# nsfisis/RayTracingInOneWeekend.zig

Hardware: AMD Instinct MI355X
Metric: Msamples/sec (pixels x spp / s), RTIOW cover scene; trace-kernel roofline (higher is better)
Workload: dtype f64; 1 GPU; BASELINE configs[1]: RTIOW cover scene 1200x675, 500 spp per GPU (500 spp frame), depth 50, rows interleaved over 1 GPU(s); width=1200, height=675, spp_frame=500, max_depth=50, seed=42, precision=f64, parallelism=rows1

## Files before the change

### include/rtw_hip.h

```cpp
#ifndef RTW_HIP_H
#define RTW_HIP_H

#include <stddef.h>
#include <stdint.h>

#ifdef __cplusplus
extern "C" {
#endif

#define RTW_ABI_VERSION 4

typedef enum {
  RTW_OK = 0,
  RTW_EINVAL = -1,
  RTW_UNSUPPORTED = -2,
  RTW_EHIP = -3,
  RTW_ENOMEM = -4,
  RTW_ENODEV = -5
} rtw_status;

typedef enum {
  RTW_LAMBERT_SOLID = 0,
  RTW_LAMBERT_CHECKER = 1,
  RTW_METAL = 2,
// ... 92 lines not shown
const char *rtw_last_error(void);

int rtw_camera_init(rtw_camera *cam, const double look_from[3], const double look_at[3],
                    const double vup[3], double vfov, double aspect_ratio, double aperture,
                    double focus_dist, double time0, double time1);
uint32_t rtw_image_height(uint32_t width, double aspect_ratio);
int rtw_cover_scene(uint64_t seed, rtw_sphere *spheres, uint32_t *n_spheres,
                    rtw_material *mats, uint32_t *n_mats, uint64_t rng_state_out[4]);

int rtw_render(const rtw_camera *cam, const rtw_sphere *spheres, uint32_t n_spheres,
               const rtw_material *mats, uint32_t n_mats, const rtw_params *params,
               uint8_t *rgb_out, float *mean_out);

typedef struct rtw_scene_s *rtw_scene;

int rtw_scene_create(const rtw_sphere *spheres, uint32_t n_spheres, const rtw_material *mats,
                     uint32_t n_mats, rtw_scene *out);
int rtw_scene_destroy(rtw_scene scene);

size_t rtw_workspace_bytes(const rtw_params *params);

typedef struct rtw_timer_s *rtw_timer;
int rtw_timer_create(rtw_timer *out);
int rtw_timer_destroy(rtw_timer t);
int rtw_timer_elapsed_ms(rtw_timer t, float *ms);

typedef struct rtw_sclk_probe_s *rtw_sclk_probe;
int rtw_sclk_probe_begin(void *stream, double wall_ms, rtw_sclk_probe *out);
int rtw_sclk_probe_end(rtw_sclk_probe p, double *mhz);

int rtw_render_device(rtw_scene scene, const rtw_camera *cam, const rtw_params *params,
                      void *workspace, size_t workspace_bytes, uint8_t *d_rgb, float *d_mean,
                      void *stream, rtw_timer timer);

int rtw_render_counts(rtw_scene scene, const rtw_camera *cam, const rtw_params *params,
                      void *workspace, size_t workspace_bytes, uint64_t counts_out[4]);
int rtw_render_counts_ex(rtw_scene scene, const rtw_camera *cam, const rtw_params *params,
                         void *workspace, size_t workspace_bytes, uint64_t counts_out[6]);
#define RTW_STATS_WORDS 16
enum {
  RTW_STAT_SAMPLES = 0, RTW_STAT_SEGMENTS = 1, RTW_STAT_F32_SKIPS = 2,
  RTW_STAT_CAND_WAVE_ITERS = 3, RTW_STAT_CAND_LANES = 4, RTW_STAT_DISC_GE0_LANES = 5,
  RTW_STAT_SPHERE_LOOP_WAVE_ITERS = 6, RTW_STAT_CULL_SURVIVOR_LANES = 7, RTW_STAT_CULL_EXACT_WAVE_ITERS = 8,
  RTW_STAT_DRAIN_SEGMENTS = 9, RTW_STAT_DRAIN_SAMPLES = 10, RTW_STAT_CLUSTER_WAVE_TESTS = 11,
  RTW_STAT_CLUSTER_WAVE_SKIPS = 12, RTW_STAT_DRAIN_WAVE_ITERS = 13,
  RTW_STAT_PRIMARY_ROUNDS = 14, RTW_STAT_PRIMARY_IDLE_LANES = 15
};
int rtw_render_stats(rtw_scene scene, const rtw_camera *cam, const rtw_params *params,
                     void *workspace, size_t workspace_bytes, uint64_t stats_out[RTW_STATS_WORDS]);
#define RTW_STATS_WORDS_EX 24
enum {
  RTW_STAT_PRIMARY_MASK_POPCOUNT = 16,
  RTW_STAT_TAIL_HELPED_SAMPLES = 17, RTW_STAT_TAIL_WAVE_ITERS = 18, RTW_STAT_TAIL_IDLE_LANE_ITERS = 19,
  RTW_STAT_UNTRACED_UNITS = 20, RTW_STAT_UNTRACED_SAMPLES = 21
};
int rtw_render_stats_ex(rtw_scene scene, const rtw_camera *cam, const rtw_params *params,
                        void *workspace, size_t workspace_bytes, uint64_t *stats_out, uint32_t n_words);


typedef enum {
  RTW_PRIM_SPHERE = 0,
  RTW_PRIM_MOVING_SPHERE = 1,
  RTW_PRIM_XY_RECT = 2,
  RTW_PRIM_XZ_RECT = 3,
  RTW_PRIM_YZ_RECT = 4
} rtw_prim_kind;

typedef struct {
  uint32_t kind, mat;
  int32_t xform;
  uint32_t reserved;
  double a[9];
} rtw_prim;

#define RTW_MAX_XFORM_OPS 4
typedef enum {
  RTW_XF_TRANSLATE = 0,
  RTW_XF_ROTATE_Y = 1
} rtw_xform_op;
typedef struct {
  uint32_t n;
  uint32_t op[RTW_MAX_XFORM_OPS];
  double v[RTW_MAX_XFORM_OPS][3];
} rtw_xform;

typedef enum {
  RTW_TEX_SOLID = 0,
  RTW_TEX_CHECKER = 1,
  RTW_TEX_NOISE = 2,
  RTW_TEX_IMAGE = 3
} rtw_texture_kind;
typedef struct {
  uint32_t kind, perlin, image, reserved;
  double color[3], odd[3], even[3];
  double scale;
} rtw_texture;

typedef enum {
  RTW_WMAT_LAMBERT = 0,
  RTW_WMAT_METAL = 1,
  RTW_WMAT_DIELECTRIC = 2,
  RTW_WMAT_LIGHT = 3
} rtw_wmaterial_kind;
typedef struct {
  uint32_t kind, tex;
  double albedo[3];
  double fuzz, ir;
// ... 175 lines not shown
```

### raytracinginoneweekend.zig_amd/csrc/rtw_capi.hip

```cpp
#include <hip/hip_runtime.h>

#include <algorithm>
#include <cstdarg>
#include <cstdio>
#include <cstdlib>
#include <cstring>
#include <map>
#include <mutex>
#include <string>
#include <utility>
#include <vector>

#include "rtw_hip.h"
#include "rtw_capi_shared.hpp"
#include "rtw_internal.hpp"
#include "rtw_math.hpp"
#include "rtw_scene_pack.hpp"

namespace {

thread_local std::string g_err;

}

int rtw_fail(int status, const char* fmt, ...) {
  char buf[512];
  va_list ap;
  va_start(ap, fmt);
  vsnprintf(buf, sizeof(buf), fmt, ap);
  va_end(ap);
  g_err = buf;
  return status;
}

namespace {

const char* dev_knob(const char* name) {
#ifdef RTW_MEASURE
  return getenv(name);
#else
  (void)name;
  return nullptr;
#endif
}

uint64_t splitmix_first(uint64_t seed) {
  uint64_t z = seed + 0x9e3779b97f4a7c15ULL;
  z = (z ^ (z >> 30)) * 0xbf58476d1ce4e5b9ULL;
  z = (z ^ (z >> 27)) * 0x94d049bb133111ebULL;
  return z ^ (z >> 31);
}

constexpr int kBpcTail = 16;
struct DevInfo {
  int cus = 0;
  std::map<std::pair<int, bool>, std::pair<size_t, int>> bpc;
};
std::mutex g_dev_mu;
std::map<int, DevInfo> g_dev;

int device_cus(int dev) {
  std::lock_guard<std::mutex> lk(g_dev_mu);
  auto& d = g_dev[dev];
  if (d.cus == 0) {
    int v = 0;
    if (hipDeviceGetAttribute(&v, hipDeviceAttributeMultiprocessorCount, dev) != hipSuccess || v <= 0) v = 256;
    d.cus = v;
// ... 157 lines not shown
  a.chunk = rtwp::eff_chunk(p);
  a.n_chunks = rtwp::n_chunks(p);
  a.row_begin = p->row_begin;
  a.row_stride = p->row_stride;
  a.row_count = p->row_count;
  a.tiles_x = rtwp::tiles_x(p);
  a.total_units = (uint32_t)rtwp::total_units(p);
  const rtwm::UDivMagic mu = rtwm::udiv_magic((uint32_t)rtwp::tile_units(1, a.n_chunks)), mt = rtwm::udiv_magic(a.tiles_x);
  a.upt_m = mu.m, a.upt_sh = mu.sh, a.tx_m = mt.m, a.tx_sh = mt.sh;
  a.seed_base = splitmix_first(p->seed) + seed_adv;
  a.unit_order = unit_order(0u);
  a.empty_on = 0u;
  a.partial = reinterpret_cast<double*>(ws + L.partial_off);
  a.counter = reinterpret_cast<uint32_t*>(ws + L.counter_off);
  a.stats = reinterpret_cast<unsigned long long*>(ws + L.stats_off);
}

size_t lds_bytes(const rtw_scene_s* sc, int prec, uint32_t n_clusters) {
  const size_t r = prec == 1 ? 4 : 8;
  return rtwk::kCoopLdsBytes + r * (8 * ((size_t)sc->n + 1) + (size_t)sc->n + 8 * (size_t)sc->nm + 4 * (size_t)sc->ng) +
         4 * ((size_t)sc->n + 1 + sc->nm + sc->n + rtwk::kClusterSlots * (size_t)n_clusters) + 16;
}

uint32_t clusters_usable(const rtw_scene_s* sc, const rtw_camera* cam) {
  if (!sc->v64.cluster_on) return 0u;
  for (const auto& g : sc->groups)
    if (!(cam->time0 >= g.first && cam->time1 <= g.second)) return 0u;
  return 1u;
}

template <typename R>
int launch_engine(const rtwk::SceneView<R>& view, const rtw_camera* cam, const rtw_params* p, unsigned char* ws,
                  const WsLayout& L, uint64_t seed_adv, const RtwPassMap& map, uint32_t cl_on, int dev, size_t lds,
                  uint32_t grid_cap, hipStream_t stream, int mode, bool masked, size_t tail_lds) {
  rtwk::TraceArgs<R> a;
  fill_args(a, view, cam, p, ws, L, seed_adv);
  map.apply(a);
  a.sc.cluster_on = cl_on;
  if (!cl_on) a.sc.n_clusters = 0u;
  a.primary_on = (p->engine == RTW_ENGINE_MEGAKERNEL && rtwk::trace_primary_first((int)p->precision, masked) &&
                  cl_on && a.sc.n_clusters * rtwk::kClusterSlots <= 64u)
                     ? 1u
                     : 0u;
  a.tail_on = (a.primary_on && tail_lds) ? 1u : 0u;
  const uint32_t n_wide = a.sc.g_static_wide + (a.sc.g_moving_wide - a.sc.g_static);
  a.empty_on = (a.primary_on && a.max_depth >= 1u && a.sc.n_clusters * rtwk::kClusterSlots + n_wide <= 64u) ? 1u : 0u;
  if (const char* ek = dev_knob("RTW_TRACE_EMPTY"); ek && ek[0] == '0') a.empty_on = 0u;
  if (a.tail_on) lds += tail_lds;
  if (p->engine == RTW_ENGINE_WAVEFRONT) {
    if (mode == 2) return rtw_fail(RTW_UNSUPPORTED, "phase profile runs on the megakernel engine");
    return rtw_run_wavefront<R>(a, p, ws, L, dev, lds, stream, mode == 1);
  }
  const uint32_t grid = std::max(1u, std::min(grid_cap, (a.total_units + 255) / 256));
  hipError_t e;
  if constexpr (sizeof(R) == 8)
    e = rtwk::launch_trace_f64(a, grid, lds, stream, mode, masked);
  else
    e = rtwk::launch_trace_f32(a, grid, lds, stream, mode, masked);
  if (e != hipSuccess) return rtw_fail(RTW_EHIP, "trace kernel launch: %s", hipGetErrorString(e));
  return RTW_OK;
}

int launch_all(rtw_scene sc, const rtw_camera* cam, const rtw_params* p, void* workspace, size_t ws_bytes,
               uint8_t* d_rgb, float* d_mean, hipStream_t stream, rtw_timer timer, int mode,
               uint64_t seed_adv = 0, rtw_accum acc = nullptr) {
  const WsLayout L = rtwp::ws_layout(p);
  int dev = 0;
  RtwPassMap map;
  bool launch = true;
  const int st0 = rtw_launch_begin(L, workspace, ws_bytes, sc->device,
                                   "scene lives on device %d but the current device is %d", acc, timer, stream, &dev,
                                   &map, &launch);
  if (st0 != RTW_OK || !launch) return st0;
  auto* ws = static_cast<unsigned char*>(workspace);
  const bool masked = map.list && p->engine == RTW_ENGINE_MEGAKERNEL;
  const uint32_t cl_on = p->precision == RTW_PRECISION_F64 ? clusters_usable(sc, cam) : 0u;
  size_t lds = lds_bytes(sc, (int)p->precision, cl_on ? sc->v64.n_clusters : 0u);
  if (p->engine == RTW_ENGINE_MEGAKERNEL) lds += rtwk::trace_home_lds_bytes((int)p->precision, masked);
  if (lds > 64 * 1024) return rtw_fail(RTW_UNSUPPORTED, "scene tables need %zu B of LDS", lds);
  const int bpc = blocks_per_cu(dev, (int)p->precision, lds, masked);
  const uint32_t grid_cap = (uint32_t)(device_cus(dev) * bpc);
  size_t tail_lds = p->engine == RTW_ENGINE_MEGAKERNEL ? rtwk::trace_tail_lds_bytes((int)p->precision, masked) : 0;
  if (const char* tk = dev_knob("RTW_TRACE_TAIL"); tk && tk[0] == '0') tail_lds = 0;
  if (tail_lds && (lds + tail_lds > 64 * 1024 || blocks_per_cu(dev, (int)p->precision, lds + tail_lds, masked, true) != bpc))
    tail_lds = 0;
  if (timer) HIP_TRY(hipEventRecord(timer->start, stream));
  const int st = p->precision == RTW_PRECISION_F32
                     ? launch_engine(sc->v32, cam, p, ws, L, seed_adv, map, cl_on, dev, lds, grid_cap, stream, mode,
                                     masked, tail_lds)
                     : launch_engine(sc->v64, cam, p, ws, L, seed_adv, map, cl_on, dev, lds, grid_cap, stream, mode,
                                     masked, tail_lds);
  if (st != RTW_OK) return st;
  if (timer) {
    HIP_TRY(hipEventRecord(timer->stop, stream));
    timer->recorded = true;
  }
  if (acc) return rtw_accum_pass_fold(acc, p, ws, stream);
  if (d_rgb) return rtw_launch_finalize(p, ws, d_rgb, d_mean, stream);
  return RTW_OK;
}
}

extern "C" {

size_t rtw_workspace_bytes(const rtw_params* p) {
  if (rtw_validate_params(p) != RTW_OK) return 0;
// ... 327 lines not shown
```

### raytracinginoneweekend.zig_amd/csrc/rtw_device.hpp

```cpp
#pragma once
#include <hip/hip_runtime.h>

#include "rtw_beam.hpp"
#include "rtw_cull.hpp"
#include "rtw_internal.hpp"
#include "rtw_math.hpp"

namespace rtwk {

template <typename R>
struct V3 {
  R x, y, z;
};
template <typename R>
__device__ __forceinline__ V3<R> mk(R x, R y, R z) {
  return V3<R>{x, y, z};
}
template <typename R>
__device__ __forceinline__ V3<R> add(V3<R> a, V3<R> b) {
  return mk(a.x + b.x, a.y + b.y, a.z + b.z);
}
template <typename R>
__device__ __forceinline__ V3<R> sub(V3<R> a, V3<R> b) {
  return mk(a.x - b.x, a.y - b.y, a.z - b.z);
// ... 550 lines not shown
      root = (-hb + sq) / a;
      if (root < tmin || tmax < root) continue;
    }
    tmax = root;
    hit = (int)k;
  }
  (void)l_rad;
}

template <typename R>
struct LdsTables {
  CoopSlots* slots;
  R* sph;
  R* rad;
  R* mat;
  R* tg;
  uint32_t* meta;
  uint32_t* kind;
  uint32_t* perm;
  uint32_t* cpos;
};
template <typename R>
__device__ __forceinline__ LdsTables<R> stage_tables(const SceneView<R>& S, unsigned char* lds_raw) {
  LdsTables<R> T;
  T.slots = reinterpret_cast<CoopSlots*>(lds_raw) + (threadIdx.x >> 6);
  T.sph = reinterpret_cast<R*>(lds_raw + kCoopBytesPerWave * (kTraceBlock / 64));
  T.rad = T.sph + 8 * (S.n + 1);
  T.mat = T.rad + S.n;
  T.tg = T.mat + 8 * S.nm;
  T.meta = reinterpret_cast<uint32_t*>(T.tg + 4 * S.ng);
  T.kind = T.meta + S.n + 1;
  T.perm = T.kind + S.nm;
  T.cpos = T.perm + S.n;
  for (uint32_t i = threadIdx.x; i < 8 * (S.n + 1); i += blockDim.x) T.sph[i] = S.sph[i];
  for (uint32_t i = threadIdx.x; i < S.n; i += blockDim.x) T.rad[i] = S.rad[i];
  for (uint32_t i = threadIdx.x; i < 8 * S.nm; i += blockDim.x) T.mat[i] = S.mat[i];
  for (uint32_t i = threadIdx.x; i < 4 * S.ng; i += blockDim.x) T.tg[i] = S.tg[i];
  for (uint32_t i = threadIdx.x; i < S.n + 1; i += blockDim.x) T.meta[i] = S.meta[i];
  for (uint32_t i = threadIdx.x; i < S.nm; i += blockDim.x) T.kind[i] = S.kind[i];
  for (uint32_t i = threadIdx.x; i < S.n; i += blockDim.x) T.perm[i] = S.perm[i];
  for (uint32_t i = threadIdx.x; i < kClusterSlots * S.n_clusters; i += blockDim.x) T.cpos[i] = S.cpos[i];
  __syncthreads();
  return T;
}

struct KStats {
  unsigned long long samples = 0, segments = 0, skipped = 0;
  unsigned long long candwave = 0, candlane = 0, disc = 0, wave_iters = 0;
  unsigned long long cull_lanes = 0, cull_iters = 0;
  unsigned long long cl_tests = 0, cl_skips = 0;
  unsigned long long prim_rounds = 0, prim_idle = 0, mask_pop = 0;
  unsigned long long tail_helped = 0, tail_iters = 0, tail_idle = 0;
  unsigned long long empty_units = 0, empty_samples = 0;
  uint64_t ph[10] = {0, 0, 0, 0, 0, 0, 0, 0, 0, 0};
  uint64_t t_last = 0;
};
#define RTW_STAMP(slot)                                                          \
  if constexpr (MODE == 2) {                                                     \
    __builtin_amdgcn_sched_barrier(0);                                           \
    uint64_t t_;                                                                 \
    asm volatile("s_memtime %0\n\ts_waitcnt lgkmcnt(0)" : "=s"(t_)::"memory"); \
    __builtin_amdgcn_sched_barrier(0);                                           \
    st.ph[slot] += t_ - st.t_last;                                               \
    st.t_last = t_;                                                              \
  }

template <typename R, bool F32, int MODE, bool PRIMARY = false, bool FLAT = false, typename SV>
__device__ __forceinline__ void closest_hit(const SV& S, const LdsTables<R>& T, const Lane<R>& L, R tmin,
                                            R pre_k, uint32_t lid, KStats& st, int& hit, R& tmax, uint32_t pm0 = 0u,
                                            uint32_t pm1 = 0u) {
  static_assert(!PRIMARY || !F32, "the primary form is f64 only (clustered tables)");
  constexpr bool STATS = MODE == 1;
  const R a = norm2(L.d);
  const R inv_a = (R)1 / a;
  const R pre_lim = pre_k * a;
  int tg_cur = -1;
  R frac = (R)0;
  const RTW_CONST uint32_t* c_meta = cptr(S.meta);
  const RTW_CONST R* c_sph = cptr(S.sph);
  const RTW_CONST R* c_tg = cptr(S.tg);
  int hit_orig = -1;
  bool nan_seen = false;
  auto accept = [&](R root, int pos, int orig) {
    if (root != root) nan_seen = true;
    if (!(root < tmin) & ((root < tmax) | ((root == tmax) & (orig > hit_orig)))) {
      tmax = root;
      hit = pos;
      hit_orig = orig;
    }
  };
  auto test = [&](uint32_t k, uint32_t meta, R cx, R cy, R cz, R r2) {
    const R ocx = L.o.x - cx, ocy = L.o.y - cy, ocz = L.o.z - cz;
    const R hb = ocx * L.d.x + ocy * L.d.y + ocz * L.d.z;
    const R cc = (ocx * ocx + ocy * ocy + ocz * ocz) - r2;
    const R disc = hb * hb - a * cc;
    if (!(disc < (R)0)) {
      const bool pre = (hb > (R)0) & (cc > (R)0) & (hb < pre_lim);
      bool cand = !pre;
      if (F32) cand = cand & ((int)k != L.skip);
      if constexpr (STATS) {
        const uint64_t cm = __ballot(cand);
        if (cm && lid == (uint32_t)__builtin_ctzll(__ballot(true))) st.candwave++;
        st.candlane += cand ? 1 : 0;
        st.disc += 1;
      }
      if (cand) {
// ... 323 lines not shown
```

### raytracinginoneweekend.zig_amd/csrc/rtw_internal.hpp

```cpp
#pragma once
#include <hip/hip_runtime.h>
#include <stdint.h>

#include "rtw_layout.hpp"

namespace rtwk {

constexpr uint32_t kBatch = 64;

template <typename R>
struct SceneView {
  const R* sph;
  const R* rad;
  const uint32_t* meta;
  const R* mat;
  const uint32_t* kind;
  const R* tg;
  const double* wide_d;
  const double* tg_d;
  const uint32_t* perm;
  const float* cull;
  const uint32_t* cull_tg;
  const float* tg_f;
  uint32_t n, nm, ng;
  uint32_t g_static_wide, g_static, g_moving_wide;
  uint32_t nn, nn_pad, n_sn;
  uint32_t cull_on;
  float cull_cmax;
  float cull_rho;
  const float* ccull;
  const uint32_t* ccull_tg;
  const float* cclus;
  const uint32_t* cpos;
  const uint32_t* cvalid;
  uint32_t n_clusters;
  uint32_t cluster_on;
  float cull_rho_cl;
};

template <typename R>
struct TraceArgs {
  SceneView<R> sc;
  R origin[3], horizontal[3], vertical[3], llc[3], cu[3], cv[3];
  R lens_radius, time0, time1;
  R bg[3];
  R tmin;
  R inv_w1, inv_h1;
  R pre_k;
  uint32_t W, H, spp, max_depth, chunk, n_chunks;
  uint32_t row_begin, row_stride, row_count, tiles_x;
  uint32_t total_units;
  uint32_t upt_m, upt_sh, tx_m, tx_sh;
  uint32_t unit_order;
  uint32_t primary_on;
  uint32_t tail_on;
  uint32_t empty_on;
  uint64_t seed_base;
  double* partial;
  uint32_t* counter;
  unsigned long long* stats;
  const uint32_t* tile_list;
  const uint64_t* tile_mask;
};

struct FinalizeArgs {
  const double* partial;
  uint8_t* rgb;
  float* mean;
  uint32_t npix, n_chunks;
  double scale;
};

hipError_t launch_trace_f64(const TraceArgs<double>& a, uint32_t grid, size_t lds, hipStream_t s, int mode,
                            bool masked);
hipError_t launch_trace_f32(const TraceArgs<float>& a, uint32_t grid, size_t lds, hipStream_t s, int mode,
                            bool masked);
hipError_t launch_finalize(const FinalizeArgs& a, hipStream_t s);
int trace_blocks_per_cu(int precision, size_t lds, bool masked);
bool trace_primary_first(int precision, bool masked);
constexpr size_t kHomeLdsBytesPerWave = 2560;
constexpr size_t kPrimaryLdsBytesPerWave = 4 * 64 * 4;
size_t trace_home_lds_bytes(int precision, bool masked);
constexpr int kTraceBlock = 256;
constexpr uint32_t kTailWindow = 4;
constexpr size_t kTailLdsBytesPerWave = (3 + kTailWindow) * 64 * 4;
size_t trace_tail_lds_bytes(int precision, bool masked);

struct FoldArgs {
  const double* partial;
  double* sum;
  double* stat;
  uint32_t npix, n_chunks;
  uint32_t n_full;
};
struct ResolveArgs {
  const double* sum;
  uint8_t* rgb;
  float* mean;
  uint32_t npix;
  double scale;
};
struct NoiseArgs {
  const double* stat;
  double* part;
  uint32_t npix;
  double m;
  double denom;
};
struct MaskedFoldArgs {
  FoldArgs f;
  const uint8_t* act;
  uint32_t* cnt;
  uint32_t pass_spp;
};
struct ActiveArgs {
  uint8_t* act;
  const uint8_t* user;
  const double* stat;
  const uint32_t* cnt;
  uint64_t* tile_mask;
  uint32_t* tile_list;
  uint32_t* n_active;
  uint32_t W, rows, tiles_x, n_tiles;
  uint32_t chunk, min_spp;
  double thr;
  uint32_t done;
  uint32_t from_cnt;
};
struct ResolveCntArgs {
  const double* sum;
  const uint32_t* cnt;
  uint8_t* rgb;
  float* mean;
  uint32_t npix;
// ... 137 lines not shown
```

### raytracinginoneweekend.zig_amd/csrc/rtw_trace.hip

```cpp
#include <hip/hip_runtime.h>

#include <type_traits>

#include "rtw_device.hpp"


namespace rtwk {

template <bool F32, bool MASKED>
struct TraceCfg {
  static constexpr int kWavesPerSimd = (F32 && !MASKED) ? 5 : 4;
  static constexpr bool kLoopArgsFromKernarg = !F32;
  static constexpr bool kPrimaryFirst = !F32 && !MASKED;
  static constexpr size_t kHomeStride = kHomeLdsBytesPerWave + (kPrimaryFirst ? kPrimaryLdsBytesPerWave : 0);
  static constexpr size_t kTailBytes = kPrimaryFirst ? kTailLdsBytesPerWave : 0;
};

template <typename R, bool F32, int MODE, bool MASKED>
__global__ void __launch_bounds__(kTraceBlock, (TraceCfg<F32, MASKED>::kWavesPerSimd)) trace_kernel(TraceArgs<R> A) {
  using Cfg = TraceCfg<F32, MASKED>;
  constexpr bool STATS = MODE == 1;
  extern __shared__ __align__(16) unsigned char lds_raw[];
  const SceneView<R> S = A.sc;
  const LdsTables<R> T = stage_tables<R>(S, lds_raw);
  CoopSlots* slots = T.slots;

  const uint32_t lid = lane_id();
  double* h_sum = nullptr;
  uint32_t* h_u32 = nullptr;
  {
    const size_t off = (size_t)(reinterpret_cast<unsigned char*>(T.cpos + kClusterSlots * S.n_clusters) - lds_raw);
    const size_t stride = Cfg::kHomeStride + (Cfg::kTailBytes != 0 && A.tail_on ? Cfg::kTailBytes : 0);
    unsigned char* hb = lds_raw + ((off + 7) & ~(size_t)7) + (threadIdx.x >> 6) * stride;
    h_sum = reinterpret_cast<double*>(hb);
    h_u32 = reinterpret_cast<uint32_t*>(hb + 3 * 64 * 8);
  }
#define RTW_KA(f) (Cfg::kLoopArgsFromKernarg ? opaque(kargs<R>())->f : A.f)
  const R kInf = (R)__builtin_huge_val();

  Lane<R> L;
  L.px = L.ly = L.s = L.depth = 0;
  L.rs = 0;
  L.skip = -1;
  uint32_t lane_flags = 0u;
  LaneFlag<1u> have_unit{lane_flags};
  LaneFlag<2u> have_ray{lane_flags};
  LaneFlag<4u> done{lane_flags};
  uint32_t qnext = 0, qend = 0;
  KStats st;
  if constexpr (MODE == 2) asm volatile("s_memtime %0\n\ts_waitcnt lgkmcnt(0)" : "=s"(st.t_last)::"memory");

  constexpr uint32_t kPm = 4 * 64, kBm = 6 * 64;
  uint32_t* const h_me = h_u32 + lid;
  constexpr bool PF = Cfg::kPrimaryFirst;
  uint32_t nb_tx = 0, nb_ty = 0, nb_c = 0;
  uint64_t nb_pad = 0;
  auto decode_batch = [&](uint32_t base, uint32_t& tx, uint32_t& ty, uint32_t& c, uint64_t& pad) {
    const uint32_t b64 = (uint32_t)__builtin_amdgcn_readfirstlane((int)(base >> 6));
    const uint32_t nc = RTW_KA(n_chunks), txs = RTW_KA(tiles_x);
    const uint32_t tile = b64 / nc;
    c = b64 - tile * nc;
    ty = tile / txs;
    tx = tile - ty * txs;
  };
  auto take_units = [&]() {
    const bool need = !have_unit && !done;
    const uint64_t needmask = __ballot(need);
    if (needmask) {
      const uint32_t n = (uint32_t)__popcll(needmask);
      const uint32_t rank = mbcnt64(needmask);
      const uint32_t rem = qend - qnext;
      uint32_t base2 = 0;
      uint32_t nb_bm0 = 0u, nb_bm1 = 0u;
      if (n > rem) for (;;) {
        uint32_t b = 0;
        if (lid == 0) b = atomicAdd(RTW_KA(counter), kBatch);
        if constexpr (PF)
          base2 = (uint32_t)__builtin_amdgcn_ds_bpermute(0, (int)b);
        else
          base2 = __shfl(b, 0);
        if constexpr (!PF) {
          break;
        } else {
          decode_batch(dealt_unit(base2, *opaque(kargs<R>())) & ~63u, nb_tx, nb_ty, nb_c, nb_pad);
          if (!RTW_KA(primary_on)) break;
          const auto* ka = opaque(kargs<R>());
          const double org[3] = {ka->origin[0], ka->origin[1], ka->origin[2]};
          const double llc[3] = {ka->llc[0], ka->llc[1], ka->llc[2]};
          const double hor[3] = {ka->horizontal[0], ka->horizontal[1], ka->horizontal[2]};
          const double ver[3] = {ka->vertical[0], ka->vertical[1], ka->vertical[2]};
          const double cu[3] = {ka->cu[0], ka->cu[1], ka->cu[2]}, cv[3] = {ka->cv[0], ka->cv[1], ka->cv[2]};
          const uint32_t px0 = nb_tx * kTileW, ly0 = nb_ty * kTileH;
          const uint32_t px1 = min(px0 + (kTileW - 1u), ka->W - 1u), ly1 = min(ly0 + (kTileH - 1u), ka->row_count - 1u);
          const rtwb::Beam beam =
              rtwb::tile_beam(org, llc, hor, ver, cu, cv, ka->lens_radius, ka->W, ka->H, px0, px1,
                              ka->row_begin + ly0 * ka->row_stride, ka->row_begin + ly1 * ka->row_stride);
          bool may = false;
          const uint32_t n_slots = kClusterSlots * ka->sc.n_clusters;
          const uint32_t n_wide = ka->empty_on ? ka->sc.g_static_wide + (ka->sc.g_moving_wide - ka->sc.g_static) : 0u;
          if (lid < n_slots + n_wide) {
            uint32_t slot = lid;
            asm volatile("" : "+v"(slot));
            const uint32_t w = lid - n_slots;
            const uint32_t k = lid < n_slots ? T.cpos[slot]
                                             : (w < ka->sc.g_static_wide ? w : ka->sc.g_static + (w - ka->sc.g_static_wide));
            const uint32_t meta = T.meta[k];
            const bool mv = (meta & kMoving) != 0;
            const uint32_t g = mv ? (meta >> 2) & 63u : 0u;
            const double g0 = mv ? (double)T.tg[4 * g] : 0.0, g1 = mv ? (double)T.tg[4 * g + 1] : 1.0;
            const double c0[3] = {(double)T.sph[8 * k], (double)T.sph[8 * k + 1], (double)T.sph[8 * k + 2]};
            const double dc[3] = {(double)T.sph[8 * k + 3], (double)T.sph[8 * k + 4], (double)T.sph[8 * k + 5]};
            may = rtwb::beam_may_hit(beam, c0, dc, (double)T.rad[k], mv, g0, g1, ka->time0, ka->time1);
          }
          const uint64_t bal = wballot(may && lid < n_slots);
          nb_bm0 = __builtin_bitreverse32((uint32_t)bal);
          nb_bm1 = __builtin_bitreverse32((uint32_t)(bal >> 32));
          const RTW_CONST uint32_t* cval = cptr(ka->sc.cvalid);
          if constexpr (STATS) {
            if (lid == 0 && base2 < RTW_KA(total_units)) st.mask_pop += __popc(nb_bm0 & cval[0]) + __popc(nb_bm1 & cval[1]);
          }
          if (!ka->empty_on || base2 >= RTW_KA(total_units)) break;
          if (((nb_bm0 & cval[0]) | (nb_bm1 & cval[1])) != 0u || wballot(may && lid >= n_slots) != 0ull) break;
          {
            const uint32_t l = dealt_unit(base2 + lid, *ka) & 63u;
            const uint32_t px = nb_tx * kTileW + (l & 7u), ly = nb_ty * kTileH + (l >> 3);
            if (px < ka->W && ly < ka->row_count) {
              const uint32_t s0 = nb_c * ka->chunk, ns = min(s0 + ka->chunk, ka->spp) - s0;
              const double bg0 = (double)ka->bg[0], bg1 = (double)ka->bg[1], bg2 = (double)ka->bg[2];
              double z = 0.0;
              asm volatile("" : "+v"(z));
              double e0 = z, e1 = z, e2 = z;
#pragma unroll 1
              for (uint32_t i = 0; i < ns; ++i) e0 += bg0, e1 += bg1, e2 += bg2;
              double* dst = ka->partial + ((size_t)nb_c * (ka->row_count * ka->W) + (size_t)ly * ka->W + px) * 3;
              dst[0] = e0;
              dst[1] = e1;
              dst[2] = e2;
              if constexpr (STATS) st.samples += ns, st.segments += ns, st.empty_units++, st.empty_samples += ns;
            }
          }
        }
      }
      if (need) {
        const uint32_t unit = rank < rem ? qnext + rank : base2 + (rank - rem);
        if (unit >= RTW_KA(total_units)) {
          done = true;
        } else {
          const uint32_t du = dealt_unit(unit, *opaque(kargs<R>()));
          const uint32_t l = du & 63u;
          bool active = true;
          const uint32_t units_per_tile = kTileW * kTileH * RTW_KA(n_chunks);
          uint32_t tile = rtwm::udiv(du, RTW_KA(upt_m), RTW_KA(upt_sh));
          const uint32_t r = du - tile * units_per_tile;
          const uint32_t c = r >> 6;
          if constexpr (MASKED) {
            const auto* ka = opaque(kargs<R>());
            tile = ka->tile_list[tile & 0xFFFFFFu] & 0xFFFFFFu;
            const uint32_t half = reinterpret_cast<const uint32_t*>(ka->tile_mask)[2u * tile + (l >> 5)];
            active = ((half >> (l & 31u)) & 1u) != 0;
          }
          const uint32_t ty = rtwm::udiv(tile, RTW_KA(tx_m), RTW_KA(tx_sh));
          const uint32_t tx = tile - ty * RTW_KA(tiles_x);
          const uint32_t px = tx * kTileW + (l & 7u);
          const uint32_t ly = ty * kTileH + (l >> 3);
          if (px < RTW_KA(W) && ly < RTW_KA(row_count) && active) {
            have_unit = true;
            L.s = c * RTW_KA(chunk);
            double z = 0.0;
            asm volatile("" : "+v"(z));
            h_u32[lid] = px;
            h_u32[64 + lid] = ly;
            h_u32[128 + lid] = c;
            h_u32[192 + lid] = min(L.s + RTW_KA(chunk), RTW_KA(spp));
            h_sum[lid] = h_sum[64 + lid] = h_sum[128 + lid] = z;
            if constexpr (PF) {
// ... 261 lines not shown
      RTW_STAMP(7)
      if (shading) {
        if (scatter_hit<R, F32, true>(T, L, hit, tmax, kind, pt, raw)) finish_sample();
      }
      if (ns) {
        if constexpr (LDISK) {
          R dk[2];
          for (;;) {
            dk[0] = rrange_m11<R>(L.rs);
            dk[1] = rrange_m11<R>(L.rs);
            if (in_unit_ball<R, 2>(dk)) break;
          }
          start_sample_ray<R>(kargs<R>(), L, u, v, dk[0], dk[1]);
        } else {
          start_sample_ray<R, true>(kargs<R>(), L, u, v, pt[0], pt[1], raw);
        }
        have_ray = true;
      }
      RTW_STAMP(8)
      shading = false;
      hit = -1;
      tmax = kInf;
      bool ended = false;
      if (have_ray) {
        const int b = bounce(kind, hit, tmax, std::false_type{});
        ended = b == 1;
        shading = b == 2;
      }
      RTW_STAMP(3)
      if (ended) finish_sample();
    }
  }
  if (STATS) {
    atomicAdd(A.stats + 0, st.samples);
    atomicAdd(A.stats + 1, st.segments);
    atomicAdd(A.stats + 2, st.skipped);
    atomicAdd(A.stats + 3, st.candwave);
    atomicAdd(A.stats + 4, st.candlane);
    atomicAdd(A.stats + 5, st.disc);
    atomicAdd(A.stats + 6, st.wave_iters);
    atomicAdd(A.stats + 7, st.cull_lanes);
    atomicAdd(A.stats + 8, st.cull_iters);
    atomicAdd(A.stats + 11, st.cl_tests);
    atomicAdd(A.stats + 12, st.cl_skips);
    if constexpr (PF) {
      atomicAdd(A.stats + 14, st.prim_rounds);
      atomicAdd(A.stats + 15, st.prim_idle);
      atomicAdd(A.stats + 16, st.mask_pop);
      atomicAdd(A.stats + 17, st.tail_helped);
      atomicAdd(A.stats + 18, st.tail_iters);
      atomicAdd(A.stats + 19, st.tail_idle);
      atomicAdd(A.stats + 20, st.empty_units);
      atomicAdd(A.stats + 21, st.empty_samples);
    }
  }
  if constexpr (MODE == 2) {
    RTW_STAMP(4)
    if (lid == 0)
      for (int i = 0; i < 10; ++i) atomicAdd(A.stats + 16 + i, (unsigned long long)st.ph[i]);
  }
}

__global__ void __launch_bounds__(256) finalize_kernel(FinalizeArgs F) {
  for (uint32_t i = blockIdx.x * blockDim.x + threadIdx.x; i < F.npix; i += gridDim.x * blockDim.x) {
    double t[3] = {0.0, 0.0, 0.0};
    for (uint32_t c = 0; c < F.n_chunks; ++c) {
      const double* p = F.partial + ((size_t)c * F.npix + i) * 3;
      t[0] += p[0];
      t[1] += p[1];
      t[2] += p[2];
    }
#pragma unroll
    for (int k = 0; k < 3; ++k) {
      const double g = sqrt(t[k] * F.scale);
      const double cl = fmax(0.0, fmin(g, 0.999));
      F.rgb[(size_t)i * 3 + k] = (uint8_t)(256.0 * cl);
      if (F.mean) F.mean[(size_t)i * 3 + k] = (float)(t[k] * F.scale);
    }
  }
}

template <typename R, bool F32>
static hipError_t launch_trace(const TraceArgs<R>& a, uint32_t grid, size_t lds, hipStream_t s, int mode,
                               bool masked) {
  if (masked) {
    if (mode != 0 || !a.tile_list || !a.tile_mask) return hipErrorInvalidValue;
    hipLaunchKernelGGL((trace_kernel<R, F32, 0, true>), dim3(grid), dim3(kTraceBlock), lds, s, a);
  } else if (mode == 1) {
    hipLaunchKernelGGL((trace_kernel<R, F32, 1, false>), dim3(grid), dim3(kTraceBlock), lds, s, a);
#ifdef RTW_MEASURE
  } else if (mode == 2) {
    hipLaunchKernelGGL((trace_kernel<R, F32, 2, false>), dim3(grid), dim3(kTraceBlock), lds, s, a);
#endif
  } else {
    hipLaunchKernelGGL((trace_kernel<R, F32, 0, false>), dim3(grid), dim3(kTraceBlock), lds, s, a);
  }
  return hipGetLastError();
}

hipError_t launch_trace_f64(const TraceArgs<double>& a, uint32_t grid, size_t lds, hipStream_t s, int mode,
                            bool masked) {
  return launch_trace<double, false>(a, grid, lds, s, mode, masked);
}
hipError_t launch_trace_f32(const TraceArgs<float>& a, uint32_t grid, size_t lds, hipStream_t s, int mode,
                            bool masked) {
  return launch_trace<float, true>(a, grid, lds, s, mode, masked);
// ... 37 lines not shown
```

### raytracinginoneweekend.zig_amd/rtw_amd/__init__.py

```python
from __future__ import annotations

import ctypes as C
import os
import re

import numpy as np

PKG_DIR = os.path.dirname(os.path.abspath(__file__))
ROOT = os.path.dirname(PKG_DIR)
REPO = os.path.dirname(ROOT)
LIB_PATH = os.environ.get("RTW_LIB_PATH") or os.path.join(ROOT, "lib", "librtw_hip.so")
HEADER_PATH = os.path.join(REPO, "include", "rtw_hip.h")

RTW_OK, RTW_EINVAL, RTW_UNSUPPORTED, RTW_EHIP, RTW_ENOMEM, RTW_ENODEV = 0, -1, -2, -3, -4, -5
LAMBERT_SOLID, LAMBERT_CHECKER, METAL, DIELECTRIC, DIFFUSE_LIGHT = 0, 1, 2, 3, 4
PRECISION = {"f64": 0, "f32": 1}
ENGINE = {"megakernel": 0, "wavefront": 1}
DEFAULT_WF_PATHS = 5 << 17
DEFAULT_WF_SETS = 2
DEFAULT_WF_PASSES = 16
WF_DRAIN = {"samples": 0, "slots": 1, "none": 2}
WF_FORM = {"fused": 0, "split": 1}
WORLD_FEATURES = {"auto": 0, "all": 1}
WORLD_TRAVERSAL = {"auto": 0, "union": 1, "lane": 2}
STATS_WORDS = 16
STAT_NAMES = ["samples", "segments", "f32_skips", "cand_wave_iters", "cand_lanes", "disc_ge0_lanes",
              "sphere_loop_wave_iters", "cull_survivor_lanes", "cull_exact_wave_iters", "drain_segments",
              "drain_samples", "cluster_wave_tests", "cluster_wave_skips", "drain_wave_iters", "primary_rounds",
              "primary_idle_lanes"]
STAT_NAMES_EX = STAT_NAMES + ["primary_mask_popcount", "tail_helped_samples", "tail_wave_iters",
                              "tail_idle_lane_iters", "untraced_units", "untraced_samples"]
DEFAULT_CHUNK = 20
COVER_BACKGROUND = (0.70, 0.80, 1.00)


class RtwError(RuntimeError):
    def __init__(self, status: int, msg: str):
        super().__init__(f"rtw status {status}: {msg}")
        self.status = status


class Material(C.Structure):
    _fields_ = [("kind", C.c_uint32), ("reserved", C.c_uint32), ("albedo", C.c_double * 3),
                ("albedo_odd", C.c_double * 3), ("fuzz", C.c_double), ("ir", C.c_double)]


class Sphere(C.Structure):
    _fields_ = [("c0", C.c_double * 3), ("c1", C.c_double * 3), ("radius", C.c_double),
                ("t0", C.c_double), ("t1", C.c_double), ("moving", C.c_uint32), ("mat", C.c_uint32)]


class Camera(C.Structure):
    _fields_ = [(n, C.c_double * 3) for n in
                ("origin", "horizontal", "vertical", "lower_left_corner", "u", "v", "w")] + \
               [("lens_radius", C.c_double), ("time0", C.c_double), ("time1", C.c_double)]


class Params(C.Structure):
    _fields_ = [("width", C.c_uint32), ("height", C.c_uint32), ("spp", C.c_uint32),
                ("max_depth", C.c_uint32), ("seed", C.c_uint64), ("background", C.c_double * 3),
                ("row_begin", C.c_uint32), ("row_stride", C.c_uint32), ("row_count", C.c_uint32),
                ("chunk", C.c_uint32), ("precision", C.c_uint32), ("device", C.c_int32),
                ("engine", C.c_uint32), ("wf_paths", C.c_uint32),
                ("wf_sets", C.c_uint32), ("wf_drain", C.c_uint32), ("wf_form", C.c_uint32),
                ("world_waves", C.c_uint32), ("world_features", C.c_uint32), ("world_traversal", C.c_uint32),
                ("wf_bounces", C.c_uint32), ("wf_passes", C.c_uint32)]


class Guide(C.Structure):
    _fields_ = [("normal", C.c_float * 3), ("depth", C.c_float), ("albedo", C.c_float * 3), ("prim", C.c_uint32)]


GUIDE_DTYPE = np.dtype([("normal", np.float32, 3), ("depth", np.float32), ("albedo", np.float32, 3),
                        ("prim", np.uint32)])
VAR_UNKNOWN, VAR_EMPTY = -1.0, -2.0
DENOISE_NO_COLOR, DENOISE_DIRECT, DENOISE_SPATIAL_VAR = 1, 2, 4


class Ray(C.Structure):
    _fields_ = [("origin", C.c_double * 3), ("dir", C.c_double * 3), ("time", C.c_double), ("t_min", C.c_double),
                ("t_max", C.c_double)]


class Hit(C.Structure):
# ... 514 lines not shown
```

Baseline: 14990 Msamples/s.

## Claim multiple work batches per atomic and cache tile beam-test results

Lets a wave reserve several consecutive 64-unit batches with a single global atomicAdd once it has seen a run of empty (miss-everything) tiles. The claim size follows a guided schedule that shrinks as the remaining work falls. The per-tile beam/cluster mask and its empty flag are cached in per-wave LDS words, so consecutive batches from the same tile skip recomputing the beam test. The aim is to cut atomic contention and redundant beam culling on the sky-only tiles. In exchange it adds a little LDS per wave, extra LDS traffic and some load-balance risk near the end of the queue.

```diff
diff --git a/include/rtw_hip.h b/include/rtw_hip.h
--- a/include/rtw_hip.h
+++ b/include/rtw_hip.h
@@ -168,7 +168,8 @@
 enum {
   RTW_STAT_PRIMARY_MASK_POPCOUNT = 16,
   RTW_STAT_TAIL_HELPED_SAMPLES = 17, RTW_STAT_TAIL_WAVE_ITERS = 18, RTW_STAT_TAIL_IDLE_LANE_ITERS = 19,
-  RTW_STAT_UNTRACED_UNITS = 20, RTW_STAT_UNTRACED_SAMPLES = 21
+  RTW_STAT_UNTRACED_UNITS = 20, RTW_STAT_UNTRACED_SAMPLES = 21,
+  RTW_STAT_QUEUE_CLAIMS = 22, RTW_STAT_BEAM_PASSES = 23
 };
 int rtw_render_stats_ex(rtw_scene scene, const rtw_camera *cam, const rtw_params *params,
                         void *workspace, size_t workspace_bytes, uint64_t *stats_out, uint32_t n_words);
diff --git a/raytracinginoneweekend.zig_amd/csrc/rtw_capi.hip b/raytracinginoneweekend.zig_amd/csrc/rtw_capi.hip
--- a/raytracinginoneweekend.zig_amd/csrc/rtw_capi.hip
+++ b/raytracinginoneweekend.zig_amd/csrc/rtw_capi.hip
@@ -13,6 +13,7 @@
 
 #include "rtw_hip.h"
 #include "rtw_capi_shared.hpp"
+#include "rtw_claim.hpp"
 #include "rtw_internal.hpp"
 #include "rtw_math.hpp"
 #include "rtw_scene_pack.hpp"
@@ -276,6 +277,9 @@
     return rtw_run_wavefront<R>(a, p, ws, L, dev, lds, stream, mode == 1);
   }
   const uint32_t grid = std::max(1u, std::min(grid_cap, (a.total_units + 255) / 256));
+  const uint32_t claim_waves = rtwc::kClaimDiv * grid * (uint32_t)(rtwk::kTraceBlock / 64);
+  a.claim_waves = (a.empty_on && a.total_units / rtwk::kBatch >= 2u * claim_waves) ? claim_waves : 0u;
+  if (const char* ck = dev_knob("RTW_TRACE_CLAIM"); ck && ck[0] == '1') a.claim_waves = 0u;
   hipError_t e;
   if constexpr (sizeof(R) == 8)
     e = rtwk::launch_trace_f64(a, grid, lds, stream, mode, masked);
diff --git a/raytracinginoneweekend.zig_amd/csrc/rtw_claim.hpp b/raytracinginoneweekend.zig_amd/csrc/rtw_claim.hpp
--- /dev/null
+++ b/raytracinginoneweekend.zig_amd/csrc/rtw_claim.hpp
@@ -0,0 +1,53 @@
+#pragma once
+#include <cstdint>
+
+#if defined(__HIPCC__)
+#define RTWC_HD __host__ __device__ __forceinline__
+#else
+#define RTWC_HD inline
+#endif
+
+namespace rtwc {
+
+constexpr uint32_t kClaimBatch = 64;
+#ifndef RTW_CLAIM_MAX
+#define RTW_CLAIM_MAX 8
+#endif
+#ifndef RTW_CLAIM_DIV
+#define RTW_CLAIM_DIV 2
+#endif
+constexpr uint32_t kClaimMax = RTW_CLAIM_MAX;
+constexpr uint32_t kClaimDiv = RTW_CLAIM_DIV;
+
+struct Reserve {
+  uint32_t next = 0, end = 0;
+};
+
+RTWC_HD uint32_t guided_k(uint32_t head, uint32_t total_units, uint32_t div_waves) {
+  if (div_waves == 0u) return 1u;
+  const uint32_t left = head < total_units ? (total_units - head) / kClaimBatch : 0u;
+  uint32_t k = 1u;
+  for (uint32_t j = 2u; j <= kClaimMax; ++j) k += left >= j * div_waves ? 1u : 0u;
+  return k;
+}
+
+RTWC_HD Reserve after_claim(uint32_t base, uint32_t k) { return {base, base + k * kClaimBatch}; }
+
+RTWC_HD bool reserve_has(const Reserve& r) { return r.next < r.end; }
+
+RTWC_HD Reserve after_fetch(const Reserve& r, uint32_t base, uint32_t total_units) {
+  return {base < total_units ? base + kClaimBatch : r.end, r.end};
+}
+
+constexpr uint32_t kNoPass = 0x7FFFFFFFu;
+RTWC_HD uint32_t pass_word(uint32_t tile, uint32_t empty) { return (tile & 0x7FFFFFFFu) | (empty << 31); }
+RTWC_HD uint32_t pass_empty(uint32_t word) { return word >> 31; }
+RTWC_HD uint32_t run_after(uint32_t run, uint32_t empty) { return empty ? (run < kClaimMax ? run + 1u : run) : 0u; }
+RTWC_HD uint32_t claim_k(uint32_t run, uint32_t head, uint32_t total_units, uint32_t div_waves) {
+  if (run < 2u) return 1u;
+  const uint32_t g = guided_k(head, total_units, div_waves);
+  return run < g ? run : g;
+}
+RTWC_HD bool same_tile(uint32_t tile, uint32_t word) { return tile == (word & 0x7FFFFFFFu); }
+
+}
diff --git a/raytracinginoneweekend.zig_amd/csrc/rtw_device.hpp b/raytracinginoneweekend.zig_amd/csrc/rtw_device.hpp
--- a/raytracinginoneweekend.zig_amd/csrc/rtw_device.hpp
+++ b/raytracinginoneweekend.zig_amd/csrc/rtw_device.hpp
@@ -626,6 +626,7 @@
   unsigned long long prim_rounds = 0, prim_idle = 0, mask_pop = 0;
   unsigned long long tail_helped = 0, tail_iters = 0, tail_idle = 0;
   unsigned long long empty_units = 0, empty_samples = 0;
+  unsigned long long claims = 0, beam_passes = 0;
   uint64_t ph[10] = {0, 0, 0, 0, 0, 0, 0, 0, 0, 0};
   uint64_t t_last = 0;
 };
diff --git a/raytracinginoneweekend.zig_amd/csrc/rtw_internal.hpp b/raytracinginoneweekend.zig_amd/csrc/rtw_internal.hpp
--- a/raytracinginoneweekend.zig_amd/csrc/rtw_internal.hpp
+++ b/raytracinginoneweekend.zig_amd/csrc/rtw_internal.hpp
@@ -55,6 +55,7 @@
   uint32_t primary_on;
   uint32_t tail_on;
   uint32_t empty_on;
+  uint32_t claim_waves;
   uint64_t seed_base;
   double* partial;
   uint32_t* counter;
@@ -79,7 +80,8 @@
 int trace_blocks_per_cu(int precision, size_t lds, bool masked);
 bool trace_primary_first(int precision, bool masked);
 constexpr size_t kHomeLdsBytesPerWave = 2560;
-constexpr size_t kPrimaryLdsBytesPerWave = 4 * 64 * 4;
+constexpr size_t kClaimLdsBytesPerWave = 32;
+constexpr size_t kPrimaryLdsBytesPerWave = 4 * 64 * 4 + kClaimLdsBytesPerWave;
 size_t trace_home_lds_bytes(int precision, bool masked);
 constexpr int kTraceBlock = 256;
 constexpr uint32_t kTailWindow = 4;
diff --git a/raytracinginoneweekend.zig_amd/csrc/rtw_trace.hip b/raytracinginoneweekend.zig_amd/csrc/rtw_trace.hip
--- a/raytracinginoneweekend.zig_amd/csrc/rtw_trace.hip
+++ b/raytracinginoneweekend.zig_amd/csrc/rtw_trace.hip
@@ -2,6 +2,7 @@
 
 #include <type_traits>
 
+#include "rtw_claim.hpp"
 #include "rtw_device.hpp"
 
 
@@ -53,6 +54,16 @@
   constexpr uint32_t kPm = 4 * 64, kBm = 6 * 64;
   uint32_t* const h_me = h_u32 + lid;
   constexpr bool PF = Cfg::kPrimaryFirst;
+  constexpr uint32_t kRs = 8 * 64;
+  auto claim_words = [&]() __attribute__((always_inline)) -> uint32_t* {
+    uint32_t l = lid;
+    asm volatile("" : "+v"(l));
+    return h_me - l + kRs;
+  };
+  if constexpr (PF) {
+    uint32_t* const cwd = claim_words();
+    cwd[0] = 0u, cwd[1] = 0u, cwd[2] = rtwc::kNoPass, cwd[5] = 0u;
+  }
   uint32_t nb_tx = 0, nb_ty = 0, nb_c = 0;
   uint64_t nb_pad = 0;
   auto decode_batch = [&](uint32_t base, uint32_t& tx, uint32_t& ty, uint32_t& c, uint64_t& pad) {
@@ -63,7 +74,7 @@
     ty = tile / txs;
     tx = tile - ty * txs;
   };
-  auto take_units = [&]() {
+  auto take_units = [&]() __attribute__((always_inline)) {
     const bool need = !have_unit && !done;
     const uint64_t needmask = __ballot(need);
     if (needmask) {
@@ -72,55 +83,86 @@
       const uint32_t rem = qend - qnext;
       uint32_t base2 = 0;
       uint32_t nb_bm0 = 0u, nb_bm1 = 0u;
+      uint32_t nb_empty = 0u;
       if (n > rem) for (;;) {
         uint32_t b = 0;
-        if (lid == 0) b = atomicAdd(RTW_KA(counter), kBatch);
-        if constexpr (PF)
-          base2 = (uint32_t)__builtin_amdgcn_ds_bpermute(0, (int)b);
-        else
+        if constexpr (!PF) {
+          if (lid == 0) b = atomicAdd(RTW_KA(counter), kBatch);
           base2 = __shfl(b, 0);
-        if constexpr (!PF) {
           break;
         } else {
+          const uint32_t cw = RTW_KA(claim_waves);
+          uint32_t* const cwd = claim_words();
+          rtwc::Reserve rs;
+          if (cw != 0u) rs.next = cwd[0], rs.end = cwd[1];
+          if (!rtwc::reserve_has(rs)) {
+            const uint32_t k = cw != 0u ? rtwc::claim_k(cwd[5], rs.end, RTW_KA(total_units), cw) : 1u;
+            if (lid == 0) b = atomicAdd(RTW_KA(counter), k * kBatch);
+            rs = rtwc::after_claim((uint32_t)__builtin_amdgcn_ds_bpermute(0, (int)b), k);
+            if constexpr (STATS) {
+              if (lid == 0) st.claims++;
+            }
+          }
+          base2 = rs.next;
+          if (cw != 0u) {
+            rs = rtwc::after_fetch(rs, base2, RTW_KA(total_units));
+            cwd[0] = rs.next, cwd[1] = rs.end;
+          }
           decode_batch(dealt_unit(base2, *opaque(kargs<R>())) & ~63u, nb_tx, nb_ty, nb_c, nb_pad);
           if (!RTW_KA(primary_on)) break;
           const auto* ka = opaque(kargs<R>());
-          const double org[3] = {ka->origin[0], ka->origin[1], ka->origin[2]};
-          const double llc[3] = {ka->llc[0], ka->llc[1], ka->llc[2]};
-          const double hor[3] = {ka->horizontal[0], ka->horizontal[1], ka->horizontal[2]};
-          const double ver[3] = {ka->vertical[0], ka->vertical[1], ka->vertical[2]};
-          const double cu[3] = {ka->cu[0], ka->cu[1], ka->cu[2]}, cv[3] = {ka->cv[0], ka->cv[1], ka->cv[2]};
-          const uint32_t px0 = nb_tx * kTileW, ly0 = nb_ty * kTileH;
-          const uint32_t px1 = min(px0 + (kTileW - 1u), ka->W - 1u), ly1 = min(ly0 + (kTileH - 1u), ka->row_count - 1u);
-          const rtwb::Beam beam =
-              rtwb::tile_beam(org, llc, hor, ver, cu, cv, ka->lens_radius, ka->W, ka->H, px0, px1,
-                              ka->row_begin + ly0 * ka->row_stride, ka->row_begin + ly1 * ka->row_stride);
-          bool may = false;
-          const uint32_t n_slots = kClusterSlots * ka->sc.n_clusters;
-          const uint32_t n_wide = ka->empty_on ? ka->sc.g_static_wide + (ka->sc.g_moving_wide - ka->sc.g_static) : 0u;
-          if (lid < n_slots + n_wide) {
-            uint32_t slot = lid;
-            asm volatile("" : "+v"(slot));
-            const uint32_t w = lid - n_slots;
-            const uint32_t k = lid < n_slots ? T.cpos[slot]
-                                             : (w < ka->sc.g_static_wide ? w : ka->sc.g_static + (w - ka->sc.g_static_wide));
-            const uint32_t meta = T.meta[k];
-            const bool mv = (meta & kMoving) != 0;
-            const uint32_t g = mv ? (meta >> 2) & 63u : 0u;
-            const double g0 = mv ? (double)T.tg[4 * g] : 0.0, g1 = mv ? (double)T.tg[4 * g + 1] : 1.0;
-            const double c0[3] = {(double)T.sph[8 * k], (double)T.sph[8 * k + 1], (double)T.sph[8 * k + 2]};
-            const double dc[3] = {(double)T.sph[8 * k + 3], (double)T.sph[8 * k + 4], (double)T.sph[8 * k + 5]};
-            may = rtwb::beam_may_hit(beam, c0, dc, (double)T.rad[k], mv, g0, g1, ka->time0, ka->time1);
-          }
-          const uint64_t bal = wballot(may && lid < n_slots);
-          nb_bm0 = __builtin_bitreverse32((uint32_t)bal);
-          nb_bm1 = __builtin_bitreverse32((uint32_t)(bal >> 32));
+          const uint32_t last = cwd[2];
+          if (cw != 0u && rtwc::same_tile(nb_ty * ka->tiles_x + nb_tx, last)) {
+            nb_bm0 = cwd[3], nb_bm1 = cwd[4];
+            nb_empty = rtwc::pass_empty(last);
+          } else {
+            const double org[3] = {ka->origin[0], ka->origin[1], ka->origin[2]};
+            const double llc[3] = {ka->llc[0], ka->llc[1], ka->llc[2]};
+            const double hor[3] = {ka->horizontal[0], ka->horizontal[1], ka->horizontal[2]};
+            const double ver[3] = {ka->vertical[0], ka->vertical[1], ka->vertical[2]};
+            const double cu[3] = {ka->cu[0], ka->cu[1], ka->cu[2]}, cv[3] = {ka->cv[0], ka->cv[1], ka->cv[2]};
+            const uint32_t px0 = nb_tx * kTileW, ly0 = nb_ty * kTileH;
+            const uint32_t px1 = min(px0 + (kTileW - 1u), ka->W - 1u), ly1 = min(ly0 + (kTileH - 1u), ka->row_count - 1u);
+            const rtwb::Beam beam =
+                rtwb::tile_beam(org, llc, hor, ver, cu, cv, ka->lens_radius, ka->W, ka->H, px0, px1,
+                                ka->row_begin + ly0 * ka->row_stride, ka->row_begin + ly1 * ka->row_stride);
+            bool may = false;
+            const uint32_t n_slots = kClusterSlots * ka->sc.n_clusters;
+            const uint32_t n_wide = ka->empty_on ? ka->sc.g_static_wide + (ka->sc.g_moving_wide - ka->sc.g_static) : 0u;
+            if (lid < n_slots + n_wide) {
+              uint32_t slot = lid;
+              asm volatile("" : "+v"(slot));
+              const uint32_t w = lid - n_slots;
+              const uint32_t k = lid < n_slots ? T.cpos[slot]
+                                               : (w < ka->sc.g_static_wide ? w : ka->sc.g_static + (w - ka->sc.g_static_wide));
+              const uint32_t meta = T.meta[k];
+              const bool mv = (meta & kMoving) != 0;
+              const uint32_t g = mv ? (meta >> 2) & 63u : 0u;
+              const double g0 = mv ? (double)T.tg[4 * g] : 0.0, g1 = mv ? (double)T.tg[4 * g + 1] : 1.0;
+              const double c0[3] = {(double)T.sph[8 * k], (double)T.sph[8 * k + 1], (double)T.sph[8 * k + 2]};
+              const double dc[3] = {(double)T.sph[8 * k + 3], (double)T.sph[8 * k + 4], (double)T.sph[8 * k + 5]};
+              may = rtwb::beam_may_hit(beam, c0, dc, (double)T.rad[k], mv, g0, g1, ka->time0, ka->time1);
+            }
+            const uint64_t bal = wballot(may && lid < n_slots);
+            nb_bm0 = __builtin_bitreverse32((uint32_t)bal);
+            nb_bm1 = __builtin_bitreverse32((uint32_t)(bal >> 32));
+            const RTW_CONST uint32_t* cval = cptr(ka->sc.cvalid);
+            nb_empty = (ka->empty_on && ((nb_bm0 & cval[0]) | (nb_bm1 & cval[1])) == 0u &&
+                        wballot(may && lid >= n_slots) == 0ull)
+                           ? 1u
+                           : 0u;
+            cwd[2] = rtwc::pass_word(nb_ty * ka->tiles_x + nb_tx, nb_empty);
+            cwd[3] = nb_bm0, cwd[4] = nb_bm1;
+            if constexpr (STATS) {
+              if (lid == 0 && base2 < RTW_KA(total_units)) st.beam_passes++;
+            }
+          }
           const RTW_CONST uint32_t* cval = cptr(ka->sc.cvalid);
+          if (base2 < RTW_KA(total_units)) cwd[5] = rtwc::run_after(cwd[5], nb_empty);
           if constexpr (STATS) {
             if (lid == 0 && base2 < RTW_KA(total_units)) st.mask_pop += __popc(nb_bm0 & cval[0]) + __popc(nb_bm1 & cval[1]);
           }
-          if (!ka->empty_on || base2 >= RTW_KA(total_units)) break;
-          if (((nb_bm0 & cval[0]) | (nb_bm1 & cval[1])) != 0u || wballot(may && lid >= n_slots) != 0ull) break;
+          if (nb_empty == 0u || base2 >= RTW_KA(total_units)) break;
           {
             const uint32_t l = dealt_unit(base2 + lid, *ka) & 63u;
             const uint32_t px = nb_tx * kTileW + (l & 7u), ly = nb_ty * kTileH + (l >> 3);
@@ -488,6 +530,8 @@
       atomicAdd(A.stats + 19, st.tail_idle);
       atomicAdd(A.stats + 20, st.empty_units);
       atomicAdd(A.stats + 21, st.empty_samples);
+      atomicAdd(A.stats + 22, st.claims);
+      atomicAdd(A.stats + 23, st.beam_passes);
     }
   }
   if constexpr (MODE == 2) {
diff --git a/raytracinginoneweekend.zig_amd/rtw_amd/__init__.py b/raytracinginoneweekend.zig_amd/rtw_amd/__init__.py
--- a/raytracinginoneweekend.zig_amd/rtw_amd/__init__.py
+++ b/raytracinginoneweekend.zig_amd/rtw_amd/__init__.py
@@ -29,7 +29,8 @@
               "drain_samples", "cluster_wave_tests", "cluster_wave_skips", "drain_wave_iters", "primary_rounds",
               "primary_idle_lanes"]
 STAT_NAMES_EX = STAT_NAMES + ["primary_mask_popcount", "tail_helped_samples", "tail_wave_iters",
-                              "tail_idle_lane_iters", "untraced_units", "untraced_samples"]
+                              "tail_idle_lane_iters", "untraced_units", "untraced_samples", "queue_claims",
+                              "beam_passes"]
 DEFAULT_CHUNK = 20
 COVER_BACKGROUND = (0.70, 0.80, 1.00)
 
```

Measured after the change: 15220 Msamples/s (median of 6 runs). 1.5% higher.
